# Daniel-Liu-c0deb0t/block-aligner

Hardware: AMD Instinct MI355X
Metric: GCUPS (DP cells/s) on 10 kbp DNA X-drop batch; bit-exact score+CIGAR vs AVX2 (higher is better)
Workload: dtype i16 (saturating lane scores) + i32 block offsets

## Files before the change

### block_aligner_amd/csrc/ba_driver.hpp

```cpp
#pragma once
#include "ba_device.hpp"

namespace ba {

#ifndef BA_BIG
#define BA_BIG 0
#endif
constexpr bool kBig = BA_BIG != 0;
__device__ __forceinline__ void lds_sync() {
    if (kBig) __builtin_amdgcn_fence(__ATOMIC_ACQ_REL, "workgroup");
    else __builtin_amdgcn_fence(__ATOMIC_ACQ_REL, "wavefront");
    __builtin_amdgcn_wave_barrier();
}
__device__ __forceinline__ void lds_fill0(short* a, uint32_t n) {
    for (uint32_t k = 2 * lane_id(); k < n; k += 128) *(int*)(a + k) = 0;
    lds_sync();
}
__device__ __forceinline__ void lds_copy(short* dst, const short* src, uint32_t n) {
    lds_sync();
    for (uint32_t k = 2 * lane_id(); k < n; k += 128) {
        const int v = *(const int*)(src + k);
        lds_sync();
        *(int*)(dst + k) = v;
    }
// ... 1692 lines not shown
                    pf_ok = false;
                    prev_dir = DIR_GROW;
                    block_size /= 2;
                    lds_copy(L.D_col, L.D_col + block_size, block_size); lds_copy(L.C_col, L.C_col + block_size, block_size);
                    lds_copy(L.D_row, L.D_row + block_size, block_size); lds_copy(L.R_row, L.R_row + block_size, block_size);
                    si += block_size; sj += block_size;
                    park<0>(parked, (int)si); park<1>(parked, (int)sj); park<2>(parked, off);
                    save_ckpt_borders(block_size);
                    right_max = lds_prefix_max8(L.D_col);
                    down_max = lds_prefix_max8(L.D_row);
                    if (TRACE) { park<3>(parked, (int)trace_top); park<4>(parked, (int)nblocks); }
                    y_drop_iter = 0;
                }
            }
            if (down_max > right_max) { si += STEP; dir = DIR_DOWN; }
            else { sj += STEP; dir = DIR_RIGHT; }
        }

        BA_TSTAMP(tr1);
        BA_TADD(prof, 15, tr0, tr1);
#ifdef BA_TIMING
        prof[16] += steps;
#endif
        if (TRACE && XDROP && chain && coldp()->prof) {
            uint32_t sc = 0;
            const uint32_t first = ub_nb < nblocks ? ub_nb : nblocks;
            for (uint32_t k = first + (uint32_t)lane_id(); k < nblocks; k += 64u) {
                const uint32_t* rp = (const uint32_t*)(blocks + k);
                const uint32_t hw = __hip_atomic_load(rp + 2, BA_RLX_AGENT), tb = __hip_atomic_load(rp + 3, BA_RLX_AGENT);
                if (tb & 0x40000000u) sc += (hw & 0xffffu) * (hw >> 16);
            }
#pragma unroll
            for (int d = 32; d >= 1; d >>= 1) sc += (uint32_t)__shfl_xor((int)sc, d, 64);
            if (is_lane(0) && sc) atomicAdd(coldp()->prof + 60, (unsigned long long)sc);
        }
        const uint32_t pair = (uint32_t)unpark<7>(parked), slot = (uint32_t)unpark<8>(parked);
        int score; uint32_t ri, rj;
        if (XDROP || FQE) { score = best_max; ri = (uint32_t)unpark<5>(parked); rj = (uint32_t)unpark<6>(parked); }
        else {
            lds_sync();
            if (dir == DIR_DOWN) score = off + uni((int)L.D_row[rlen - sj]) - ZERO;
            else score = off + uni((int)L.D_col[qlen - si]) - ZERO;
            ri = qlen; rj = rlen;
        }
        uint32_t ncig = 0;
        if (TRACE && batch_traceback) {
            if (is_lane(0)) {
                coldp()->score[pair] = score; coldp()->query_idx[pair] = ri; coldp()->reference_idx[pair] = rj;
                if (coldp()->cells) coldp()->cells[pair] = cells;
                if (coldp()->nblocks_out) coldp()->nblocks_out[pair] = nblocks;
                if (coldp()->trace_words_out) coldp()->trace_words_out[pair] = trace_top;
            }
            hand_off(slot, pair, ri, rj);
            return mout;
        }
        const bool walk_later = TRACE && coldp()->trace_off && qlen + rlen < coldp()->inline_len2 && !(MULTI && walk_now && !SPECIAL);
        if (TRACE && coldp()->cig_ops && !status && !walk_later) {
            __builtin_amdgcn_fence(__ATOMIC_SEQ_CST, "agent");
            if constexpr (SPECIAL) {
                if (is_lane(0)) {
                    uint32_t st = 0;
                    ncig = traceback(blocks, nblocks, trace, ri, rj, q, r, h_flags, coldp()->cig_ops, coldp()->cig_off[pair], coldp()->cig_off[pair + 1], &st);
                    status |= st;
                }
            } else {
                uint32_t st = 0;
                lds_sync();
// ... 245 lines not shown
```

### block_aligner_amd/csrc/ba_host.cpp

```cpp
#include <hip/hip_runtime.h>

#include <algorithm>
#include <functional>
#include <cmath>
#include <cstdarg>
#include <cstdio>
#include <cstdlib>
#include <cstring>
#include <map>
#include <memory>
#include <string>
#include <vector>
#include <atomic>
#include <chrono>
#include <thread>

#include "../../include/block_aligner_hip.h"
#include "aa_matrices.inc"
#include "ba_launch.h"

using ba::BatchParams;
using ba::BlockRec;

typedef const ba::KernelEntry* KernelTable[2][ba::N_KINDS][ba::N_CLASSES][ba::FAM_COUNT];
// ... 1707 lines not shown
    HIP_TRY(hipSetDevice(b->device));
    if (b->compacted && b->retried == 0) {
        const unsigned long long total = *(volatile unsigned long long*)b->h_total;
        if (total <= b->compact_used_cap) {
            if (total > capacity) return fail("cigar buffer too small: need %llu entries", total);
            if (b->compact_host) { if (runs != b->compact_host && total) memcpy(runs, b->compact_host, total * 4); }
            else if (total) HIP_TRY(hipMemcpy(runs, b->compact.p, total * 4, hipMemcpyDeviceToHost));
            return 0;
        }
    }
    std::vector<uint32_t> len(b->n);
    if (d2h(b->cig_len, len.data(), b->n)) return 1;
    std::vector<uint64_t> out_off(b->n);
    uint64_t total = 0;
    if (b->h_order.empty()) for (uint32_t p = 0; p < b->n; p++) { out_off[p] = total; total += len[p]; }
    else {
        std::vector<uint32_t> dev_of(b->n);
        for (uint32_t s = 0; s < b->n; s++) dev_of[b->h_order[s]] = s;
        for (uint32_t p = 0; p < b->n; p++) { out_off[dev_of[p]] = total; total += len[dev_of[p]]; }
    }
    if (total > capacity) return fail("cigar buffer too small: need %llu entries", (unsigned long long)total);
    if (total == 0) return 0;
    DevBuf d_off, d_out;
    if (d_off.alloc(b->n * 8) || d_out.alloc(total * 4)) return 1;
    HIP_TRY(hipMemcpy(d_off.p, out_off.data(), b->n * 8, hipMemcpyHostToDevice));
    HIP_TRY(ba_launch_compact_cigars(b->stream, b->cig_ops.as<uint32_t>(), b->cig_off.as<uint64_t>(), b->cig_len.as<uint32_t>(),
                                     d_off.as<uint64_t>(), d_out.as<uint32_t>(), b->n));
    HIP_TRY(hipStreamSynchronize(b->stream));
    HIP_TRY(hipMemcpy(runs, d_out.p, total * 4, hipMemcpyDeviceToHost));
    return 0;
}
#ifdef BA_DEV
int ba_dev_lane_scan(int form, const int16_t* x, uint32_t n_cells, int gap_extend, int16_t* out) {
    if (form < 0 || form > 4 || !x || !out) return fail("ba_dev_lane_scan: bad arguments");
    const uint32_t per_wave = form <= 1 ? 512u : (form == 2 ? 128u : (form == 3 ? 64u : 32u));
    if (n_cells == 0 || n_cells % per_wave) return fail("ba_dev_lane_scan: %u cells are not whole waves of %u", n_cells, per_wave);
    if (gap_extend > 0 || gap_extend < -128) return fail("ba_dev_lane_scan: gap_extend %d", gap_extend);
    DevBuf dx, dout;
    if (dx.alloc((size_t)n_cells * 2) || dout.alloc((size_t)n_cells * 2)) return 1;
    HIP_TRY(hipMemcpy(dx.p, x, (size_t)n_cells * 2, hipMemcpyHostToDevice));
    HIP_TRY(ba_launch_lane_kat(nullptr, form, dx.as<short>(), dout.as<short>(), gap_extend, n_cells / per_wave));
    HIP_TRY(hipDeviceSynchronize());
    HIP_TRY(hipMemcpy(out, dout.p, (size_t)n_cells * 2, hipMemcpyDeviceToHost));
    return 0;
}
int ba_dev_kernel_forms(int family, int kind, int pclass, int special) {
    const ba::KernelEntry* k = find_kernel(family, kind, pclass, special);
    return !k ? 0 : (k->fn[1][0][0] ? 2 : 1);
}
#endif
int ba_batch_prof(BaBatch* b, uint64_t out[128]) {
    if (!b) return fail("null batch");
    HIP_TRY(hipMemcpy(out, b->prof.p, 1024, hipMemcpyDeviceToHost));
    return 0;
}
int ba_batch_info(BaBatch* b, uint64_t out[4]) {
    if (!b) return fail("null batch");
    out[0] = (uint64_t)b->grid * b->wpw; out[1] = b->lds / b->wpw; out[2] = b->trace.bytes; out[3] = b->pool_bytes;
    return 0;
}
int ba_batch_spec_cells(BaBatch* b, uint64_t* cells) {
    if (!b || !cells) return fail("null argument");
    if (!b->ran) return fail("ba_batch_run has not been called");
    HIP_TRY(hipSetDevice(b->device));
    HIP_TRY(hipMemcpy(cells, (const char*)b->prof.p + 60 * 8, 8, hipMemcpyDeviceToHost));
    return 0;
}
int ba_batch_kernel(BaBatch* b) {
// ... 975 lines not shown
```

### block_aligner_amd/csrc/ba_kernels.hip

```cpp
#include "ba_driver.hpp"
#include "ba_launch.h"

#ifndef BA_KIND
#error "define BA_KIND"
#endif
#ifndef BA_PMAX
#error "define BA_PMAX"
#endif

#ifndef BA_SPECIAL
#define BA_SPECIAL 0
#endif

#if !BA_BIG && (BA_KIND != 3 || (!BA_SPECIAL && BA_PMAX <= 8))
#include "ba_multi.hpp"
#endif
#if !BA_BIG && BA_PMAX <= 8 && (BA_KIND != 3 || !BA_SPECIAL)
#include "ba_small.hpp"
#endif
#if !BA_BIG && BA_PMAX == 1 && !BA_SPECIAL
#include "ba_quad.hpp"
#endif

#define K_ALIGN(T, X) ba::k_align<BA_PMAX, BA_KIND, T, X, (BA_SPECIAL != 0)>
// ... 31 lines not shown
    BA_ENTRY(ba::FAM_SMALL, ba::WAVES_PER_WG, K_SMALL),
#endif
#if BA_SPECIAL && !BA_BIG && BA_KIND != 3
    BA_ENTRY_SPM(ba::FAM_MULTI, ba::WAVES_PER_WG, K_MULTI_S1, K_MULTI_S2),
#endif
#if BA_SPECIAL && !BA_BIG && BA_PMAX <= 8 && BA_KIND != 3
    BA_ENTRY_SPM(ba::FAM_SMALL, ba::WAVES_PER_WG, K_SMALL_S1, K_SMALL_S2),
#endif
#if BA_PMAX == 1 && !BA_SPECIAL && !BA_BIG
    {ba::FAM_QUAD, ba::WAVES_PER_WG, ba::lds_table_bytes_h(BA_KIND) + ba::WAVES_PER_WG * 4 * ba::QUAD_SLOT_BYTES, {BA_TX(K_QUAD), {}}},
#endif
};
[[maybe_unused]] static const int g_registered = ba::register_kernels(BA_KIND, BA_PMAX, BA_SPECIAL != 0, g_entries, (int)(sizeof g_entries / sizeof g_entries[0]));

#if BA_KIND == 0 && BA_PMAX == 1 && !BA_SPECIAL && !BA_BIG
__global__ void __launch_bounds__(64) k_traceback(const ba::BatchParams bp) {
    using namespace ba;
    __shared__ uint32_t words[4096];
    uint32_t st = 0, n = 0;
    if (bp.flags & (F_LOCAL | F_FQS)) {
        if (lane_id() == 0)
            n = traceback(bp.blocks + (uint64_t)bp.tb_slot * bp.blocks_stride, bp.tb_nblocks, bp.trace_arena + (uint64_t)bp.tb_slot * bp.trace_stride, bp.tb_i,
                          bp.tb_j, bp.pool + bp.q_off[0], bp.pool + bp.r_off[0], bp.flags, bp.cig_ops, bp.cig_off[0], bp.cig_off[1], &st);
    } else
        n = walk_wave<false>(bp.blocks + (uint64_t)bp.tb_slot * bp.blocks_stride, bp.tb_nblocks, bp.trace_arena + (uint64_t)bp.tb_slot * bp.trace_stride, bp.tb_i,
                             bp.tb_j, bp.pool + bp.q_off[0], bp.pool + bp.r_off[0], (bp.flags & F_CIGAR_EQ) != 0, bp.cig_ops, bp.cig_off[0], bp.cig_off[1], &st,
                             words, 4096u);
    if (lane_id() == 0) { bp.cig_len[0] = n; bp.status[0] = st; }
}

__global__ void __launch_bounds__(64) k_lane_kat(int form, const short* __restrict__ x, short* __restrict__ out, int gap_extend) {
    using namespace ba;
    const int lane = lane_id();
    if (form <= 1) {
        const short* xi = x + (size_t)blockIdx.x * 512 + lane * 8;
        int xr[4], r[4];
#pragma unroll
        for (int k = 0; k < 4; k++) xr[k] = pk((int)xi[2 * k], (int)xi[2 * k + 1]);
        const int ge2 = splat(gap_extend);
#pragma unroll
        for (int k = 0; k < 4; k++) r[k] = scan8_inreg(xr[k], ge2);
        int G[4], cs;
        if (form == 0) {
            const MultiConsts mc = make_multi_consts(lane & 15, gap_extend);
#pragma unroll
            for (int k = 0; k < 4; k++) G[k] = mc.G[k];
            scan8_chain(r, G[0]);
            cs = multi_carry(r[3], mc);
        } else {
            const SmallConsts mc = make_small_consts(lane & 3, gap_extend);
#pragma unroll
            for (int k = 0; k < 4; k++) G[k] = mc.G[k];
            scan8_chain(r, G[0]);
            cs = small_carry(r[3], mc, lane & 3);
        }
        short* oi = out + (size_t)blockIdx.x * 512 + lane * 8;
#pragma unroll
        for (int k = 0; k < 4; k++) { const int v = scan8_apply(r[k], cs, G[k], k == 3); oi[2 * k] = as_s(v).x; oi[2 * k + 1] = as_s(v).y; }
    } else {
        const int nl = form == 2 ? 64 : (form == 3 ? 32 : 16);
        const size_t base = (size_t)blockIdx.x * (size_t)(2 * nl);
        const int xv = lane < nl ? pk((int)x[base + 2 * lane], (int)x[base + 2 * lane + 1]) : 0;
        const FillConsts fc = make_fill_consts(lane, 0, gap_extend);
        const int v = form == 2 ? fast_scan<64>(xv, fc) : (form == 3 ? fast_scan<32>(xv, fc) : fast_scan<16>(xv, fc));
        if (lane < nl) { out[base + 2 * lane] = as_s(v).x; out[base + 2 * lane + 1] = as_s(v).y; }
    }
}
extern "C" hipError_t ba_launch_lane_kat(hipStream_t s, int form, const short* x, short* out, int gap_extend, unsigned waves) {
    k_lane_kat<<<dim3(waves), dim3(64), 0, s>>>(form, x, out, gap_extend);
    return hipGetLastError();
}

constexpr int WALK_WAVES = 4;
__global__ void __launch_bounds__(WALK_WAVES * 64) k_walk(const ba::BatchParams bp) {
    extern __shared__ __attribute__((aligned(16))) unsigned char walk_lds[];
    ba::traceback_all(bp, (uint32_t)ba::F_CIGAR_EQ, walk_lds + ((uint32_t)threadIdx.x >> 6) * ba::TB_LDS_BYTES);
}

__global__ void __launch_bounds__(WALK_WAVES * 64) k_walk_l2(const ba::BatchParams bp) {
// ... 134 lines not shown
```

### block_aligner_amd/csrc/ba_multi.hpp

```cpp
#pragma once
#include "ba_quad.hpp"

namespace ba {
#ifndef MQ_SOLO_PRIO
#define MQ_SOLO_PRIO 2
#endif

template <int N>
__device__ __forceinline__ int row_bcast(int v) { return __builtin_amdgcn_update_dpp(v, v, 0x150 + N, 0xf, 0xf, false); }
__device__ __forceinline__ int row_shl1_keep(int last, int src) { return __builtin_amdgcn_update_dpp(last, src, 0x101, 0xf, 0xf, false); }
__device__ __forceinline__ int splat_hi(int x) { const s16x2 t = as_s(x); return as_i(s16x2{t.y, t.y}); }
__device__ __forceinline__ int splat_lo(int x) { const s16x2 t = as_s(x); return as_i(s16x2{t.x, t.x}); }

__device__ __forceinline__ int sel_mask(unsigned long long m, int a, int b) {
    int r;
    asm("v_cndmask_b32_e64 %0, %1, %2, %3" : "=v"(r) : "v"(b), "v"(a), "s"(m));
    return r;
}

template <int SL> __device__ __forceinline__ int slot_first(int v) {
    if constexpr (SL == 16) return row_bcast<0>(v);
    else if constexpr (SL == 64) return __builtin_amdgcn_readfirstlane(v);
    else return __builtin_amdgcn_ds_bpermute((lane_id() & 32) << 2, v);
}
template <int SL> __device__ __forceinline__ int slot_last(int v) {
    if constexpr (SL == 16) return row_bcast<15>(v);
    else if constexpr (SL == 64) return __builtin_amdgcn_readlane(v, 63);
    else return __builtin_amdgcn_ds_bpermute(((lane_id() & 32) + 31) << 2, v);
}
template <int SL> __device__ __forceinline__ int slot_shr1_z(int v, int l) {
    if constexpr (SL == 16) return row_shr1_z(v);
    else if constexpr (SL == 64) return wave_shr1_z(v);
    else { const int t = wave_shr1_z(v); return l == 0 ? 0 : t; }
}
template <int SL> __device__ __forceinline__ int slot_shl1_keep(int last, int src, int l) {
    if constexpr (SL == 16) return row_shl1_keep(last, src);
    else { const int t = __builtin_amdgcn_update_dpp(last, src, 0x130, 0xf, 0xf, false); return l == SL - 1 ? last : t; }
}

struct MultiConsts {
    int G[4];
    int laneKG, lanem1KG;
    int w0;
};

__device__ __forceinline__ MultiConsts make_multi_consts(int l, int gx) {
    MultiConsts mc;
    mc.laneKG = l * 8 * gx; mc.lanem1KG = l ? (l - 1) * 8 * gx : -32768;
#pragma unroll
    for (int k = 0; k < 4; k++) mc.G[k] = pk(max(-32768, (2 * k + 1) * gx), max(-32768, (2 * k + 2) * gx));
    mc.w0 = pk(0, l == 0 ? 0 : ((l & 1) ? max(-32768, 8 * l * gx) : 4 * gx));
    return mc;
}
template <int SL = 16>
__device__ __forceinline__ int multi_carry(int r3, const MultiConsts& mc, int l = 0) {
    if constexpr (SL == 16) {
        const int pm = wave_prefix_max16((int)as_s(r3).y - mc.laneKG);
        return vmax(scan8_splat_lo(add_row_shr1(pm, mc.lanem1KG)), mc.w0);
    } else {
        const int pm = SL == 64 ? wave_prefix_max((int)as_s(r3).y - mc.laneKG) : wave_prefix_max32((int)as_s(r3).y - mc.laneKG);
        const int cin = add_shr1(pm, mc.lanem1KG);
        return vmax(scan8_splat_lo(l == 0 ? -32768 : cin), mc.w0);
    }
}

struct MultiOut { int mx, act_max8, pas_max8, corner_new; };

template <int KIND, bool TRACE, int SPM = 0, int SL = 16>
__device__ __forceinline__ void multi_rect(const char* table, const FillConsts& fc, const MultiConsts& mc, int l, int (&Ad)[4], int (&Ac)[4],
                                           int (&Pd)[4], int (&Pr)[4], uint2 vb, uint32_t cb_lo, uint32_t cb_hi, int corner, int off_add,
                                           uint32_t* __restrict__ tout, bool store, MultiOut& o, int rz2 = 0, bool fqs_row0 = false, int* zout = nullptr) {
    uint32_t zacc[2] = {0, 0};
    const int offa = splat(off_add);
    int d[4], c[4], pd[4], pr[4];
#pragma unroll
    for (int k = 0; k < 4; k++) {
        d[k] = adds(Ad[k], offa); c[k] = adds(Ac[k], offa); pd[k] = adds(Pd[k], offa); pr[k] = adds(Pr[k], offa);
    }
    o.corner_new = slot_first<SL>(pd[3]) >> 16;
    ScoreKey<KIND> key[4];
#pragma unroll
    for (int k = 0; k < 4; k++) {
        const uint32_t w = k < 2 ? vb.x : vb.y;
        key[k] = make_key<KIND>((int)((w >> (16 * (k & 1))) & 0xffu), (int)((w >> (16 * (k & 1) + 8)) & 0xffu));
    }
    uint32_t kb[4] = {0, 0, 0, 0}, cbs_lo = 0, cbs_hi = 0;
    if constexpr (KIND == KIND_NUC) {
        const uint32_t tb = (uint32_t)(uintptr_t)table, k01 = nuc_keys2(vb.x), k23 = nuc_keys2(vb.y);
        kb[0] = add_word(k01, tb, 0); kb[1] = add_word(k01, tb, 1); kb[2] = add_word(k23, tb, 0); kb[3] = add_word(k23, tb, 1);
        cbs_lo = nuc_col_offsets(cb_lo); cbs_hi = nuc_col_offsets(cb_hi);
    }
    int dmax[4] = {0, 0, 0, 0}, tacc[8] = {0, 0, 0, 0, 0, 0, 0, 0};
    int nvD[4] = {0, 0, 0, 0}, nvR[4] = {0, 0, 0, 0};
    int holdD = 0, holdR = 0;
#pragma unroll
    for (int j = 0; j < STEP; j++) {
        const int cb = (int)(((j < 4 ? cb_lo : cb_hi) >> (8 * (j & 3))) & 0xffu);
        int sc[4];
#pragma unroll
        for (int k = 0; k < 4; k++) {
            if constexpr (KIND == KIND_NUC) sc[k] = lds_read_i32(add_byte(j < 4 ? cbs_lo : cbs_hi, kb[k], j));
            else sc[k] = fetch_score<KIND>(table, key[k], cb);
        }
        int prev = slot_shr1_z<SL>(d[3], l);
        if (j == 0) prev = l == 0 ? (int)((uint32_t)corner << 16) : prev;
        int d00[4];
        d00[0] = __builtin_amdgcn_alignbit(d[0], prev, 16);
#pragma unroll
        for (int k = 1; k < 4; k++) d00[k] = __builtin_amdgcn_alignbit(d[k], d[k - 1], 16);
        int d11[4], copen[4], cn[4], x[4], r[4];
#pragma unroll
        for (int k = 0; k < 4; k++) {
            d11[k] = adds(d00[k], sc[k]);
            if (SPM == 2 && k == 0) d11[0] = fqs_row0 ? (int)(((uint32_t)d11[0] & 0xffff0000u) | ((uint32_t)rz2 & 0xffffu)) : d11[0];
            if (SPM == 1) d11[k] = vmax(d11[k], rz2);
            copen[k] = adds(d[k], fc.go2);
            cn[k] = vmax(adds(c[k], fc.ge2), copen[k]);
            d11[k] = vmax(d11[k], cn[k]);
            x[k] = adds(d11[k], fc.ome2);
            r[k] = scan8_inreg(x[k], fc.ge2);
        }
        scan8_chain(r, mc.G[0]);
        const int cs = multi_carry<SL>(r[3], mc, l);
        int dn[4];
        uint32_t sC[4], sR[4], sCo[4], sRo[4];
#pragma unroll
        for (int k = 0; k < 4; k++) {
            r[k] = scan8_apply(r[k], cs, mc.G[k], k == 3);
            dn[k] = vmax(d11[k], r[k]);
            if (TRACE) {
                sC[k] = (uint32_t)subs(cn[k], dn[k]); sR[k] = (uint32_t)subs(r[k], dn[k]); sCo[k] = (uint32_t)subs(copen[k], cn[k]); sRo[k] = (uint32_t)subs(x[k], r[k]);
            }
            dmax[k] = vmax(dmax[k], dn[k]);
            d[k] = dn[k]; c[k] = cn[k];
        }
        if (TRACE && SPM == 1) {
#pragma unroll
            for (int p2 = 0; p2 < 2; p2++) {
                const uint32_t pZ = (uint32_t)__builtin_amdgcn_perm(subs(rz2, dn[2 * p2 + 1]), subs(rz2, dn[2 * p2]), 0x0b0a0908);
                zacc[p2] |= pZ & (0x01010101u << j);
            }
        }
        if (TRACE) {
#pragma unroll
            for (int p2 = 0; p2 < 2; p2++) {
                const uint32_t pC = (uint32_t)__builtin_amdgcn_perm((int)sC[2 * p2 + 1], (int)sC[2 * p2], 0x0b0a0908), pR = (uint32_t)__builtin_amdgcn_perm((int)sR[2 * p2 + 1], (int)sR[2 * p2], 0x0b0a0908);
                const uint32_t pCo = (uint32_t)__builtin_amdgcn_perm((int)sCo[2 * p2 + 1], (int)sCo[2 * p2], 0x0b0a0908), pRo = (uint32_t)__builtin_amdgcn_perm((int)sRo[2 * p2 + 1], (int)sRo[2 * p2], 0x0b0a0908);
                const uint32_t lo2 = bfi(0x55555555u, pC, pR), hi2 = bfi(0x55555555u, pCo, pRo);
                const uint32_t nib = bfi(0x33333333u, lo2, hi2);
                if (j & 1) tacc[2 * (j >> 1) + p2] = (int)bfi(0xF0F0F0F0u, nib, (uint32_t)tacc[2 * (j >> 1) + p2]);
                else tacc[2 * (j >> 1) + p2] = (int)nib;
            }
        }
        if (j & 1) { nvD[j >> 1] = __builtin_amdgcn_perm(dn[3], holdD, 0x07060302); nvR[j >> 1] = __builtin_amdgcn_perm(r[3], holdR, 0x07060302); }
        else { holdD = dn[3]; holdR = r[3]; }
    }
    if (TRACE) {
#ifndef MQ_X_NOTRSTORE
        if (store) { *(int4*)tout = int4{tacc[0], tacc[1], tacc[2], tacc[3]}; *(int4*)(tout + 4) = int4{tacc[4], tacc[5], tacc[6], tacc[7]}; }
#else
        asm volatile("" :: "v"(tacc[0]), "v"(tacc[1]), "v"(tacc[2]), "v"(tacc[3]), "v"(tacc[4]), "v"(tacc[5]), "v"(tacc[6]), "v"(tacc[7]));
#endif
    }
#pragma unroll
    for (int k = 0; k < 4; k++) {
        Pd[k] = slot_shl1_keep<SL>(nvD[k], pd[k], l); Pr[k] = slot_shl1_keep<SL>(nvR[k], pr[k], l);
        Ad[k] = d[k]; Ac[k] = c[k];
    }
    {
        const int ma = vmax(vmax(d[0], d[1]), vmax(d[2], d[3])), mb = vmax(vmax(Pd[0], Pd[1]), vmax(Pd[2], Pd[3]));
        const s16x2 sa = as_s(ma), sb = as_s(mb);
        const int xa = vmax(ma, as_i(s16x2{sa.y, sa.x})), xb = vmax(mb, as_i(s16x2{sb.y, sb.x}));
        const s16x2 rr = as_s(slot_first<SL>(__builtin_amdgcn_perm(xb, xa, 0x05040100)));
        o.act_max8 = rr.x; o.pas_max8 = rr.y;
    }
    const int mm = vmax(vmax(dmax[0], dmax[1]), vmax(dmax[2], dmax[3]));
    const int m32 = max(mm & 0xffff, (int)((uint32_t)mm >> 16));
    o.mx = slot_last<SL>(SL == 16 ? wave_prefix_max16(m32) : (SL == 64 ? wave_prefix_max(m32) : wave_prefix_max32(m32)));
    if constexpr (TRACE && SPM == 1) { zout[0] = (int)~zacc[0]; zout[1] = (int)~zacc[1]; }
}

enum { MR_PAIR = 0, MR_BEST_I, MR_BEST_J, MR_CELLS_LO, MR_CELLS_HI, MR_BUDGET, MR_STATUS, MR_TSLOT, MR_SI, MR_SJ, MR_DIR, MR_PREV_DIR, MR_OFF, MR_OFF_MAX,
       MR_BEST_MAX, MR_Y_DROP, MR_X_ITER, MR_D_CORNER, MR_NSTEPS, MR_TRACE_TOP, MR_NBLOCKS, MR_SEL, MR_WORDS };
__device__ __forceinline__ int mq_load(const char* p) { return __hip_atomic_load((const int*)p, BA_RLX_AGENT); }

#ifndef MQ_PARTIAL_MB
#define MQ_PARTIAL_MB 256
#endif
#ifndef MQ_WAVES_EU
#define MQ_WAVES_EU 4
#endif
template <int PMAX, int KIND, bool TRACE, bool XDROP, int SPM = 0, int MBP = 128, int WPW = WAVES_PER_WG, int EU = MQ_WAVES_EU>
__global__ void __launch_bounds__(WPW * 64, (PMAX >= 16 ? 2 : EU)) k_multi(const BatchParams bp) {
    constexpr uint32_t MB = (uint32_t)MBP;
    constexpr int SL = MBP / 8, NSLOT = 64 / SL;
    constexpr uint32_t ALLM = (1u << NSLOT) - 1u;
    constexpr uint32_t ARR = 2u * MB, BUFL = 4u * ARR, BUFA = BUFL + 64u, SLOTA = 2u * BUFA + 128u;
    static_assert((MBP == 128 || MBP == 256 || MBP == 512) && NSLOT * SLOTA <= MQ_WAVE_BYTES && NSLOT * 2u * BUFL <= MQ_LDS_SCALARS && (MBP == 128 || SPM == 0), "k_multi slot geometry");
    static_assert(MBP != 128 || (BUFA == MQ_BUF_BYTES && SLOTA == MQ_SLOT_BYTES), "ba_params.h");
    constexpr uint32_t MQ_TW = (STEP * MB / 8) * (SPM == 1 ? 2u : 1u);
    constexpr int TB_LB = SPM ? (int)TB_LANE_BYTES_LOC : (int)TB_LANE_BYTES_L2;
    constexpr uint32_t TB_MASK = SPM ? ~0u : (uint32_t)F_CIGAR_EQ;
    extern __shared__ __attribute__((aligned(16))) char smem[];
    const int lane = lane_id(), l = lane & (SL - 1), g = lane / SL;
    const int wave = uni((int)threadIdx.x >> 6);
    {
        char* tab = smem;
        if (KIND == KIND_NUC) {
            nuc_table_fill(tab, bp.matrix, (int)threadIdx.x, WPW * 64);
        } else {
            const int nbytes = KIND == KIND_AA ? 27 * 32 : 2;
            for (int k = (int)threadIdx.x; k < nbytes; k += WPW * 64) tab[k] = (char)bp.matrix[k];
// ... 286 lines not shown
            } else live_m &= ~(1u << solo);
#ifdef BA_TIMING
            t_solo += __builtin_amdgcn_s_memtime() - ts_a; n_solo++;
#endif
        }
        if (!live_m) break;

        {
            BA_TSTAMP(tq_a);
            char* const slot_mem = wave_mem + (uint32_t)g * SLOTA;
            const int x_drop = bp.x_drop;
            FillConsts fq;
            fq.go2 = splat(bp.gap_open); fq.ge2 = splat(gx); fq.ome2 = splat(clamp16(bp.gap_open - gx));
            MultiConsts mc = make_multi_consts(l, gx);
            const uint64_t tcap64 = bp.trace_stride, bcap64 = bp.blocks_stride;
            const uint32_t tcap = (uint32_t)(tcap64 < 0x7fffffffull ? tcap64 : 0x7fffffffull), bcap = (uint32_t)(bcap64 < 0x7fffffffull ? bcap64 : 0x7fffffffull);
            const bool live = (live_m >> g) & 1u;
            const char* rec = slot_mem + 2 * BUFA;
#define BA_R(k) (live ? mq_load(rec + 4 * (k)) : 0)
            const uint32_t pair = (uint32_t)BA_R(MR_PAIR), tslot = (uint32_t)BA_R(MR_TSLOT);
            uint32_t si = (uint32_t)BA_R(MR_SI), sj = (uint32_t)BA_R(MR_SJ), y_drop = (uint32_t)BA_R(MR_Y_DROP);
            uint32_t trace_top = (uint32_t)BA_R(MR_TRACE_TOP), nblocks = (uint32_t)BA_R(MR_NBLOCKS), sel = (uint32_t)BA_R(MR_SEL);
            int dir = BA_R(MR_DIR), prev_dir = BA_R(MR_PREV_DIR), off = BA_R(MR_OFF), off_max = BA_R(MR_OFF_MAX), best_max = BA_R(MR_BEST_MAX);
            int x_iter = BA_R(MR_X_ITER), D_corner = BA_R(MR_D_CORNER);
#undef BA_R
            int A_d[4], A_c[4], P_d[4], P_r[4];
            {
                const char* b = slot_mem + (sel ^ 1u) * BUFA + l * 16;
#pragma unroll
                for (int k = 0; k < 4; k++) {
                    A_d[k] = live ? mq_load(b + 4 * k) : 0; A_c[k] = live ? mq_load(b + ARR + 4 * k) : 0;
                    P_d[k] = live ? mq_load(b + 2 * ARR + 4 * k) : 0; P_r[k] = live ? mq_load(b + 3 * ARR + 4 * k) : 0;
                }
            }
            char* const lbuf = base + (uint32_t)g * (2u * BUFL);
            int* const lsc = (int*)(base + MQ_LDS_SCALARS) + (uint32_t)g * MQ_LSC_INTS;
            lds_sync();
            const unsigned long long qa_r = TRACE ? 0ull : (unsigned long long)(bp.pool + (live ? bp.q_off[pair] : 0ull)), ra_r = TRACE ? 0ull : (unsigned long long)(bp.pool + (live ? bp.r_off[pair] : 0ull));
            const uint32_t qlen_r = (!TRACE && live) ? bp.q_len[pair] : 0u, rlen_r = (!TRACE && live) ? bp.r_len[pair] : 0u;
            if (TRACE && l == 0) {
                const unsigned long long qa = (unsigned long long)(bp.pool + (live ? bp.q_off[pair] : 0ull)), ra = (unsigned long long)(bp.pool + (live ? bp.r_off[pair] : 0ull));
                *(int4*)(lsc + 20) = int4{(int)(uint32_t)qa, (int)(uint32_t)(qa >> 32), (int)(uint32_t)ra, (int)(uint32_t)(ra >> 32)};
                *(int4*)(lsc + 24) = int4{live ? (int)bp.q_len[pair] : 0, live ? (int)bp.r_len[pair] : 0, (int)tslot, 0};
            }
            if (live) {
                const char* cb = slot_mem + sel * BUFA;
                char* d = lbuf + sel * BUFL + l * 16;
#pragma unroll
                for (int a = 0; a < 4; a++) {
                    const char* sp = cb + a * ARR + l * 16;
                    *(int4*)(d + a * ARR) = int4{mq_load(sp), mq_load(sp + 4), mq_load(sp + 8), mq_load(sp + 12)};
                }
                if (l < 9) lsc[sel * 9u + l] = mq_load(cb + BUFL + 4 * l);
            }
            lds_sync();
            uint2 pf_qv = {0, 0}, pf_rv = {0, 0}, pf_qc = {0, 0}, pf_rc = {0, 0}; bool pf_ok = false;
            bool leave = false;
            auto stage = [&](uint32_t which, uint32_t s_i, uint32_t s_j, int s_off, uint32_t s_tt, uint32_t s_nb, int s_dir, int s_offadd, int s_corner) {
                char* b = lbuf + which * BUFL + l * 16;
                *(int4*)(b) = int4{A_d[0], A_d[1], A_d[2], A_d[3]}; *(int4*)(b + ARR) = int4{A_c[0], A_c[1], A_c[2], A_c[3]};
                *(int4*)(b + 2 * ARR) = int4{P_d[0], P_d[1], P_d[2], P_d[3]}; *(int4*)(b + 3 * ARR) = int4{P_r[0], P_r[1], P_r[2], P_r[3]};
                if (l == 0) {
                    int* sc = lsc + which * 9u;
                    sc[0] = 1; sc[1] = (int)s_i; sc[2] = (int)s_j; sc[3] = s_off; sc[4] = (int)s_tt; sc[5] = (int)s_nb; sc[6] = s_dir; sc[7] = s_offadd; sc[8] = s_corner;
                }
            };
            do {
                const bool right = dir == DIR_RIGHT;
                int4 cA = {0, 0, 0, 0}, cB = {0, 0, 0, 0};
                if (TRACE) { cA = *(const int4*)(lsc + 20); cB = *(const int4*)(lsc + 24); }
                const uint8_t* const qp = TRACE ? (const uint8_t*)((unsigned long long)(uint32_t)cA.x | ((unsigned long long)(uint32_t)cA.y << 32)) : (const uint8_t*)qa_r;
                const uint8_t* const rp = TRACE ? (const uint8_t*)((unsigned long long)(uint32_t)cA.z | ((unsigned long long)(uint32_t)cA.w << 32)) : (const uint8_t*)ra_r;
                const uint32_t qlen = TRACE ? (uint32_t)cB.x : qlen_r, rlen = TRACE ? (uint32_t)cB.y : rlen_r;
                const uint32_t ri = right ? si : sj, rj = (right ? sj : si) + (MB - STEP);
                const uint32_t lenV = right ? qlen : rlen, lenC = right ? rlen : qlen;
                const bool q_out = si + MB > qlen, r_out = sj + MB > rlen;
                bool elig = XDROP || ri + MB <= lenV || rj + STEP <= lenC;
                if (TRACE) elig = elig && nblocks < bcap && trace_top + MQ_TW + 64 <= tcap;
                leave = live && !elig;
                const bool run = live && !leave;
                const int off_n = off_max;
                const int off_add = sat16(off - off_n);
                const int corner = (prev_dir != dir && prev_dir != DIR_GROW) ? sat16(D_corner + off_add) : 0;
#ifndef MQ_X_NOSTAGE
                if (live) stage(sel ^ 1u, si, sj, off_n, trace_top, nblocks, dir, off_add, corner);
#endif
                asm volatile("" : "+v"(mc.laneKG), "+v"(mc.lanem1KG), "+v"(mc.w0));
                uint32_t l8;
                asm volatile("v_mbcnt_lo_u32_b32 %0, -1, 0\n\tv_mbcnt_hi_u32_b32 %0, -1, %0" : "=v"(l8));
                l8 = (l8 & (uint32_t)(SL - 1)) * 8u;
                uint2 vb, cbv;
                {
                    const uint8_t* Vp = right ? qp : rp; const uint8_t* Cp = right ? rp : qp;
                    vb = right ? pf_qv : pf_rv; cbv = right ? pf_rc : pf_qc;
                    if (__any(run && !pf_ok)) {
                        if (run && !pf_ok) {
                            const uint32_t* vp = (const uint32_t*)(Vp + (ri + l8));
                            vb.x = vp[0]; vb.y = vp[1];
                            const uint32_t* cp = (const uint32_t*)(Cp + rj);
                            cbv.x = cp[0]; cbv.y = cp[1];
                        }
                    }
                    asm volatile("" : "+v"(vb.x), "+v"(vb.y));
                    if (run) {
                        const uint32_t* a = (const uint32_t*)(qp + (si + l8)); const uint32_t* b = (const uint32_t*)(rp + (sj + l8));
                        const uint32_t* cq = (const uint32_t*)(qp + si + MB); const uint32_t* cr = (const uint32_t*)(rp + sj + MB);
                        pf_qv.x = a[0]; pf_qv.y = a[1]; pf_rv.x = b[0]; pf_rv.y = b[1];
                        pf_qc.x = cq[0]; pf_qc.y = cq[1]; pf_rc.x = cr[0]; pf_rc.y = cr[1];
                        pf_ok = true;
                    }
                }
                uint32_t* tw = nullptr;
                if (TRACE) {
                    uint32_t ts = (uint32_t)cB.z; asm volatile("" : "+v"(ts));
                    tw = bp.trace_arena + (uint64_t)ts * bp.trace_stride + (trace_top + l8);
                    if (run && l == 0) {
                        BlockRec br;
                        br.i = (right ? ri : rj) | 0x80000000u;
                        br.j = right ? rj : ri; br.h = (uint16_t)(right ? MB : STEP); br.w = (uint16_t)(right ? STEP : MB);
                        br.trace_base = trace_top | (right ? 0x80000000u : 0u);
                        bp.blocks[(uint64_t)(uint32_t)cB.z * bp.blocks_stride + nblocks] = br;
                    }
                }
// ... 5 lines not shown

                const int right_max = right ? o.act_max8 : o.pas_max8, down_max = right ? o.pas_max8 : o.act_max8;
                const int new_off_max = off_n + o.mx - ZERO;
                const bool improve = new_off_max > best_max;
                const uint32_t new_y = improve ? 0u : y_drop + 1;
                bool stop = q_out && r_out;
                if (XDROP) stop = stop || (!improve && new_off_max < best_max - x_drop && x_iter >= 1);
                stop = stop || (!q_out && !r_out && 2 * MB <= max_size && new_y > MB / STEP - 1);
                const bool commit = run && !stop;
                leave = leave || (run && stop);
                {
                    const bool imp = commit && improve;
                    if (keep_pre) sel ^= imp ? 1u : 0u;
                    best_max = imp ? new_off_max : best_max;
                    off = commit ? off_n : off; off_max = commit ? new_off_max : off_max; y_drop = commit ? new_y : y_drop;
                    prev_dir = commit ? dir : prev_dir; D_corner = commit ? o.corner_new : D_corner;
                    if (TRACE) { trace_top += commit ? MQ_TW : 0u; nblocks += commit ? 1u : 0u; }
                    if (XDROP) x_iter = commit ? ((new_off_max < best_max - x_drop) ? x_iter + 1 : 0) : x_iter;
                    const bool go_down = r_out || (!q_out && down_max > right_max);
                    si += (commit && go_down) ? (uint32_t)STEP : 0u; sj += (commit && !go_down) ? (uint32_t)STEP : 0u;
                    const int ndir = go_down ? DIR_DOWN : DIR_RIGHT;
                    const unsigned long long swap_m = __ballot(ndir != dir);
#pragma unroll
                    for (int k = 0; k < 4; k++) {
                        const int td = A_d[k], tc = A_c[k];
                        A_d[k] = sel_mask(swap_m, P_d[k], td); A_c[k] = sel_mask(swap_m, P_r[k], tc); P_d[k] = sel_mask(swap_m, td, P_d[k]); P_r[k] = sel_mask(swap_m, tc, P_r[k]);
                    }
                    dir = commit ? ndir : dir;
                }
#ifdef BA_TIMING
                n_quad++;
#endif
            } while (!__any(leave));
            if (live && !leave) stage(sel ^ 1u, si, sj, 0, trace_top, nblocks, dir, 0, 0);
            lds_sync();
            if (live) {
#pragma unroll
                for (int w = 0; w < 2; w++) {
                    const char* sp = lbuf + w * BUFL + l * 16;
                    char* d = slot_mem + w * BUFA + l * 16;
#pragma unroll
                    for (int a = 0; a < 4; a++) *(int4*)(d + a * ARR) = *(const int4*)(sp + a * ARR);
                    if (l < 9) *(int*)(slot_mem + w * BUFA + BUFL + 4 * l) = lsc[w * 9 + l];
                }
            }
            lds_sync();
            if (live && l == 0) {
                int* rc = (int*)(slot_mem + 2 * BUFA);
                const uint32_t nsteps = (uint32_t)mq_load((const char*)(rc + MR_NSTEPS)) + ((si + sj) - (uint32_t)mq_load((const char*)(rc + MR_SI)) - (uint32_t)mq_load((const char*)(rc + MR_SJ))) / (uint32_t)STEP;
                rc[MR_SI] = (int)si; rc[MR_SJ] = (int)sj; rc[MR_DIR] = dir; rc[MR_PREV_DIR] = prev_dir; rc[MR_OFF] = off; rc[MR_OFF_MAX] = off_max; rc[MR_BEST_MAX] = best_max;
                rc[MR_Y_DROP] = (int)y_drop; rc[MR_X_ITER] = x_iter; rc[MR_D_CORNER] = D_corner; rc[MR_NSTEPS] = (int)nsteps; rc[MR_TRACE_TOP] = (int)trace_top;
                rc[MR_NBLOCKS] = (int)nblocks; rc[MR_SEL] = (int)sel;
            }
            const unsigned long long lm = __ballot(leave && l == 0);
            pend_m = 0;
#pragma unroll
            for (int sl_i = 0; sl_i < NSLOT; sl_i++) pend_m |= (uint32_t)((lm >> (sl_i * SL)) & 1ull) << sl_i;
#ifdef BA_TIMING
            t_quad += __builtin_amdgcn_s_memtime() - tq_a;
#endif
        }
    }
#ifdef BA_TIMING
    if (bp.prof && is_lane(0)) {
        atomicMax(bp.prof + 40, (unsigned long long)__builtin_amdgcn_s_memrealtime());
        atomicAdd(bp.prof + 50, t_solo); atomicAdd(bp.prof + 51, t_quad); atomicAdd(bp.prof + 52, t_wait); atomicAdd(bp.prof + 53, n_solo); atomicAdd(bp.prof + 54, n_quad); atomicAdd(bp.prof + 55, 1ull);
    }
#endif
#ifdef BA_ENDHIST
    if (bp.prof && is_lane(0)) {
        const unsigned long long t0 = __hip_atomic_load(bp.prof + 43, BA_RLX_AGENT), t = __builtin_amdgcn_s_memrealtime();
        const unsigned long long k = t0 && t > t0 ? (t - t0) / 400000ull : 0ull;
        atomicAdd(bp.prof + 64 + (k < 63ull ? k : 63ull), 1ull);
        atomicMax(bp.prof + 40, t);
    }
#endif
// ... 23 lines not shown
```

Measured before the change: 2267.

## Split lane cells into even/odd half-words and restructure multi-slot scan

Changes the in-register layout of each lane's eight i16 cells so each packed register holds two cells four apart (split/join at load/store boundaries). The prefix scan along the column becomes a cross-register chain with a short cross-half fix-up, replacing the per-register in-register scan plus chain and apply steps. This should cut ALU and permute work in the hot block step. The trace packing, the key extraction and the column-value extraction are re-permuted to match. It also rewrites LDS staging through explicit address-space-3 pointers and recomputes lane addresses inside the loop. Risks include layout mismatches that would break bit-exactness.

After: 2338, median of 6. +3.1%, better.

```diff
diff --git a/block_aligner_amd/csrc/ba_driver.hpp b/block_aligner_amd/csrc/ba_driver.hpp
--- a/block_aligner_amd/csrc/ba_driver.hpp
+++ b/block_aligner_amd/csrc/ba_driver.hpp
@@ -1748,7 +1748,7 @@
             }
 #pragma unroll
             for (int d = 32; d >= 1; d >>= 1) sc += (uint32_t)__shfl_xor((int)sc, d, 64);
-            if (is_lane(0) && sc) atomicAdd(coldp()->prof + 60, (unsigned long long)sc);
+            if (is_lane(0) && sc && !(status & ST_CLASS_OVERFLOW)) atomicAdd(coldp()->prof + 60, (unsigned long long)sc);
         }
         const uint32_t pair = (uint32_t)unpark<7>(parked), slot = (uint32_t)unpark<8>(parked);
         int score; uint32_t ri, rj;
diff --git a/block_aligner_amd/csrc/ba_host.cpp b/block_aligner_amd/csrc/ba_host.cpp
--- a/block_aligner_amd/csrc/ba_host.cpp
+++ b/block_aligner_amd/csrc/ba_host.cpp
@@ -1763,8 +1763,8 @@
 }
 #ifdef BA_DEV
 int ba_dev_lane_scan(int form, const int16_t* x, uint32_t n_cells, int gap_extend, int16_t* out) {
-    if (form < 0 || form > 4 || !x || !out) return fail("ba_dev_lane_scan: bad arguments");
-    const uint32_t per_wave = form <= 1 ? 512u : (form == 2 ? 128u : (form == 3 ? 64u : 32u));
+    if (form < 0 || form > 7 || !x || !out) return fail("ba_dev_lane_scan: bad arguments");
+    const uint32_t per_wave = (form <= 1 || form >= 5) ? 512u : (form == 2 ? 128u : (form == 3 ? 64u : 32u));
     if (n_cells == 0 || n_cells % per_wave) return fail("ba_dev_lane_scan: %u cells are not whole waves of %u", n_cells, per_wave);
     if (gap_extend > 0 || gap_extend < -128) return fail("ba_dev_lane_scan: gap_extend %d", gap_extend);
     DevBuf dx, dout;
diff --git a/block_aligner_amd/csrc/ba_kernels.hip b/block_aligner_amd/csrc/ba_kernels.hip
--- a/block_aligner_amd/csrc/ba_kernels.hip
+++ b/block_aligner_amd/csrc/ba_kernels.hip
@@ -87,6 +87,22 @@
 __global__ void __launch_bounds__(64) k_lane_kat(int form, const short* __restrict__ x, short* __restrict__ out, int gap_extend) {
     using namespace ba;
     const int lane = lane_id();
+    if (form >= 5) {
+        const short* xi = x + (size_t)blockIdx.x * 512 + lane * 8;
+        int r[4];
+#pragma unroll
+        for (int k = 0; k < 4; k++) r[k] = pk((int)xi[k], (int)xi[k + 4]);
+        const int ge2 = splat(gap_extend);
+        const int l = lane & (form == 5 ? 15 : (form == 6 ? 31 : 63));
+        const MultiConsts mc = make_multi_consts(l, gap_extend);
+        const int r3 = scan_halves(r, ge2, mc);
+        const int cs = form == 5 ? multi_carry<16>(r3, mc, l) : (form == 6 ? multi_carry<32>(r3, mc, l) : multi_carry<64>(r3, mc, l));
+        apply_halves(r, r3, cs, ge2, mc);
+        short* oi = out + (size_t)blockIdx.x * 512 + lane * 8;
+#pragma unroll
+        for (int k = 0; k < 4; k++) { oi[k] = as_s(r[k]).x; oi[k + 4] = as_s(r[k]).y; }
+        return;
+    }
     if (form <= 1) {
         const short* xi = x + (size_t)blockIdx.x * 512 + lane * 8;
         int xr[4], r[4];
@@ -99,7 +115,7 @@
         if (form == 0) {
             const MultiConsts mc = make_multi_consts(lane & 15, gap_extend);
 #pragma unroll
-            for (int k = 0; k < 4; k++) G[k] = mc.G[k];
+            for (int k = 0; k < 4; k++) G[k] = pk(max(-32768, (2 * k + 1) * gap_extend), max(-32768, (2 * k + 2) * gap_extend));
             scan8_chain(r, G[0]);
             cs = multi_carry(r[3], mc);
         } else {
diff --git a/block_aligner_amd/csrc/ba_multi.hpp b/block_aligner_amd/csrc/ba_multi.hpp
--- a/block_aligner_amd/csrc/ba_multi.hpp
+++ b/block_aligner_amd/csrc/ba_multi.hpp
@@ -38,8 +38,31 @@
     else { const int t = __builtin_amdgcn_update_dpp(last, src, 0x130, 0xf, 0xf, false); return l == SL - 1 ? last : t; }
 }
 
+__device__ __forceinline__ void cells_split(int (&v)[4]) {
+    const int a = v[0], b = v[1], c = v[2], d = v[3];
+    v[0] = __builtin_amdgcn_perm(c, a, 0x05040100); v[1] = __builtin_amdgcn_perm(c, a, 0x07060302);
+    v[2] = __builtin_amdgcn_perm(d, b, 0x05040100); v[3] = __builtin_amdgcn_perm(d, b, 0x07060302);
+}
+__device__ __forceinline__ void cells_join(int (&v)[4]) {
+    const int a = v[0], b = v[1], c = v[2], d = v[3];
+    v[0] = __builtin_amdgcn_perm(b, a, 0x05040100); v[1] = __builtin_amdgcn_perm(d, c, 0x05040100);
+    v[2] = __builtin_amdgcn_perm(b, a, 0x07060302); v[3] = __builtin_amdgcn_perm(d, c, 0x07060302);
+}
+__device__ __forceinline__ int4 cells_split(int4 q) { int v[4] = {q.x, q.y, q.z, q.w}; cells_split(v); return int4{v[0], v[1], v[2], v[3]}; }
+__device__ __forceinline__ int4 cells_join(int4 q) { int v[4] = {q.x, q.y, q.z, q.w}; cells_join(v); return int4{v[0], v[1], v[2], v[3]}; }
+__device__ __forceinline__ int adds_lo(int a, int k) {
+    int t;
+    asm("v_pk_add_i16 %0, %1, %2 op_sel_hi:[0,1] clamp" : "=v"(t) : "v"(a), "s"(k));
+    return t;
+}
+__device__ __forceinline__ int max_hi_lo(int a, int b) {
+    asm("v_max_i16_sdwa %0, %0, %1 dst_sel:WORD_1 dst_unused:UNUSED_PRESERVE src0_sel:WORD_1 src1_sel:WORD_0" : "+v"(a) : "v"(b));
+    return a;
+}
+
 struct MultiConsts {
-    int G[4];
+    int g2, g3;
+    int K4, G48;
     int laneKG, lanem1KG;
     int w0;
 };
@@ -47,8 +70,8 @@
 __device__ __forceinline__ MultiConsts make_multi_consts(int l, int gx) {
     MultiConsts mc;
     mc.laneKG = l * 8 * gx; mc.lanem1KG = l ? (l - 1) * 8 * gx : -32768;
-#pragma unroll
-    for (int k = 0; k < 4; k++) mc.G[k] = pk(max(-32768, (2 * k + 1) * gx), max(-32768, (2 * k + 2) * gx));
+    mc.g2 = splat(max(-32768, 2 * gx)); mc.g3 = splat(max(-32768, 3 * gx));
+    mc.K4 = pk(0, max(-32768, 4 * gx)); mc.G48 = pk(max(-32768, 4 * gx), max(-32768, 8 * gx));
     mc.w0 = pk(0, l == 0 ? 0 : ((l & 1) ? max(-32768, 8 * l * gx) : 4 * gx));
     return mc;
 }
@@ -64,6 +87,18 @@
     }
 }
 
+__device__ __forceinline__ int scan_halves(int (&r)[4], int ge2, const MultiConsts& mc) {
+#pragma unroll
+    for (int k = 1; k < 4; k++) r[k] = vmax(r[k], adds(r[k - 1], ge2));
+    return vmax(r[3], adds_lo(r[3], mc.K4));
+}
+__device__ __forceinline__ void apply_halves(int (&r)[4], int r3, int cs, int ge2, const MultiConsts& mc) {
+    const int t = max_hi_lo(adds_lo(cs, mc.K4), r[3]);
+    r[0] = vmax(r[0], adds(t, ge2)); r[1] = vmax(r[1], adds(t, mc.g2)); r[2] = vmax(r[2], adds(t, mc.g3));
+    r[3] = vmax(r3, adds(cs, mc.G48));
+}
+
+typedef int lds_v4i __attribute__((ext_vector_type(4)));
 struct MultiOut { int mx, act_max8, pas_max8, corner_new; };
 
 template <int KIND, bool TRACE, int SPM = 0, int SL = 16>
@@ -80,19 +115,17 @@
     o.corner_new = slot_first<SL>(pd[3]) >> 16;
     ScoreKey<KIND> key[4];
 #pragma unroll
-    for (int k = 0; k < 4; k++) {
-        const uint32_t w = k < 2 ? vb.x : vb.y;
-        key[k] = make_key<KIND>((int)((w >> (16 * (k & 1))) & 0xffu), (int)((w >> (16 * (k & 1) + 8)) & 0xffu));
-    }
+    for (int k = 0; k < 4; k++) key[k] = make_key<KIND>((int)((vb.x >> (8 * k)) & 0xffu), (int)((vb.y >> (8 * k)) & 0xffu));
     uint32_t kb[4] = {0, 0, 0, 0}, cbs_lo = 0, cbs_hi = 0;
     if constexpr (KIND == KIND_NUC) {
-        const uint32_t tb = (uint32_t)(uintptr_t)table, k01 = nuc_keys2(vb.x), k23 = nuc_keys2(vb.y);
+        const uint32_t tb = (uint32_t)(uintptr_t)table;
+        const uint32_t k01 = nuc_keys2((uint32_t)__builtin_amdgcn_perm((int)vb.y, (int)vb.x, 0x05010400)), k23 = nuc_keys2((uint32_t)__builtin_amdgcn_perm((int)vb.y, (int)vb.x, 0x07030602));
         kb[0] = add_word(k01, tb, 0); kb[1] = add_word(k01, tb, 1); kb[2] = add_word(k23, tb, 0); kb[3] = add_word(k23, tb, 1);
         cbs_lo = nuc_col_offsets(cb_lo); cbs_hi = nuc_col_offsets(cb_hi);
     }
     int dmax[4] = {0, 0, 0, 0}, tacc[8] = {0, 0, 0, 0, 0, 0, 0, 0};
     int nvD[4] = {0, 0, 0, 0}, nvR[4] = {0, 0, 0, 0};
-    int holdD = 0, holdR = 0;
+    int holdD[4] = {0, 0, 0, 0}, holdR[4] = {0, 0, 0, 0};
 #pragma unroll
     for (int j = 0; j < STEP; j++) {
         const int cb = (int)(((j < 4 ? cb_lo : cb_hi) >> (8 * (j & 3))) & 0xffu);
@@ -105,9 +138,9 @@
         int prev = slot_shr1_z<SL>(d[3], l);
         if (j == 0) prev = l == 0 ? (int)((uint32_t)corner << 16) : prev;
         int d00[4];
-        d00[0] = __builtin_amdgcn_alignbit(d[0], prev, 16);
-#pragma unroll
-        for (int k = 1; k < 4; k++) d00[k] = __builtin_amdgcn_alignbit(d[k], d[k - 1], 16);
+        d00[0] = __builtin_amdgcn_alignbit(d[3], prev, 16);
+#pragma unroll
+        for (int k = 1; k < 4; k++) d00[k] = d[k - 1];
         int d11[4], copen[4], cn[4], x[4], r[4];
 #pragma unroll
         for (int k = 0; k < 4; k++) {
@@ -118,15 +151,15 @@
             cn[k] = vmax(adds(c[k], fc.ge2), copen[k]);
             d11[k] = vmax(d11[k], cn[k]);
             x[k] = adds(d11[k], fc.ome2);
-            r[k] = scan8_inreg(x[k], fc.ge2);
-        }
-        scan8_chain(r, mc.G[0]);
-        const int cs = multi_carry<SL>(r[3], mc, l);
+            r[k] = x[k];
+        }
+        const int r3 = scan_halves(r, fc.ge2, mc);
+        const int cs = multi_carry<SL>(r3, mc, l);
+        apply_halves(r, r3, cs, fc.ge2, mc);
         int dn[4];
         uint32_t sC[4], sR[4], sCo[4], sRo[4];
 #pragma unroll
         for (int k = 0; k < 4; k++) {
-            r[k] = scan8_apply(r[k], cs, mc.G[k], k == 3);
             dn[k] = vmax(d11[k], r[k]);
             if (TRACE) {
                 sC[k] = (uint32_t)subs(cn[k], dn[k]); sR[k] = (uint32_t)subs(r[k], dn[k]); sCo[k] = (uint32_t)subs(copen[k], cn[k]); sRo[k] = (uint32_t)subs(x[k], r[k]);
@@ -137,23 +170,27 @@
         if (TRACE && SPM == 1) {
 #pragma unroll
             for (int p2 = 0; p2 < 2; p2++) {
-                const uint32_t pZ = (uint32_t)__builtin_amdgcn_perm(subs(rz2, dn[2 * p2 + 1]), subs(rz2, dn[2 * p2]), 0x0b0a0908);
+                const uint32_t pZ = (uint32_t)__builtin_amdgcn_perm(subs(rz2, dn[2 * p2 + 1]), subs(rz2, dn[2 * p2]), 0x0b090a08);
                 zacc[p2] |= pZ & (0x01010101u << j);
             }
         }
         if (TRACE) {
 #pragma unroll
             for (int p2 = 0; p2 < 2; p2++) {
-                const uint32_t pC = (uint32_t)__builtin_amdgcn_perm((int)sC[2 * p2 + 1], (int)sC[2 * p2], 0x0b0a0908), pR = (uint32_t)__builtin_amdgcn_perm((int)sR[2 * p2 + 1], (int)sR[2 * p2], 0x0b0a0908);
-                const uint32_t pCo = (uint32_t)__builtin_amdgcn_perm((int)sCo[2 * p2 + 1], (int)sCo[2 * p2], 0x0b0a0908), pRo = (uint32_t)__builtin_amdgcn_perm((int)sRo[2 * p2 + 1], (int)sRo[2 * p2], 0x0b0a0908);
+                const uint32_t pC = (uint32_t)__builtin_amdgcn_perm((int)sC[2 * p2 + 1], (int)sC[2 * p2], 0x0b090a08), pR = (uint32_t)__builtin_amdgcn_perm((int)sR[2 * p2 + 1], (int)sR[2 * p2], 0x0b090a08);
+                const uint32_t pCo = (uint32_t)__builtin_amdgcn_perm((int)sCo[2 * p2 + 1], (int)sCo[2 * p2], 0x0b090a08), pRo = (uint32_t)__builtin_amdgcn_perm((int)sRo[2 * p2 + 1], (int)sRo[2 * p2], 0x0b090a08);
                 const uint32_t lo2 = bfi(0x55555555u, pC, pR), hi2 = bfi(0x55555555u, pCo, pRo);
                 const uint32_t nib = bfi(0x33333333u, lo2, hi2);
                 if (j & 1) tacc[2 * (j >> 1) + p2] = (int)bfi(0xF0F0F0F0u, nib, (uint32_t)tacc[2 * (j >> 1) + p2]);
                 else tacc[2 * (j >> 1) + p2] = (int)nib;
             }
-        }
-        if (j & 1) { nvD[j >> 1] = __builtin_amdgcn_perm(dn[3], holdD, 0x07060302); nvR[j >> 1] = __builtin_amdgcn_perm(r[3], holdR, 0x07060302); }
-        else { holdD = dn[3]; holdR = r[3]; }
+            if (j & 1) {
+                const int wa = tacc[j - 1], wb = tacc[j];
+                tacc[j - 1] = __builtin_amdgcn_perm(wb, wa, 0x05040100); tacc[j] = __builtin_amdgcn_perm(wb, wa, 0x07060302);
+            }
+        }
+        if (j >= 4) { nvD[j - 4] = __builtin_amdgcn_perm(dn[3], holdD[j - 4], 0x07060302); nvR[j - 4] = __builtin_amdgcn_perm(r[3], holdR[j - 4], 0x07060302); }
+        else { holdD[j] = dn[3]; holdR[j] = r[3]; }
     }
     if (TRACE) {
 #ifndef MQ_X_NOTRSTORE
@@ -177,7 +214,7 @@
     const int mm = vmax(vmax(dmax[0], dmax[1]), vmax(dmax[2], dmax[3]));
     const int m32 = max(mm & 0xffff, (int)((uint32_t)mm >> 16));
     o.mx = slot_last<SL>(SL == 16 ? wave_prefix_max16(m32) : (SL == 64 ? wave_prefix_max(m32) : wave_prefix_max32(m32)));
-    if constexpr (TRACE && SPM == 1) { zout[0] = (int)~zacc[0]; zout[1] = (int)~zacc[1]; }
+    if constexpr (TRACE && SPM == 1) { zout[0] = ~__builtin_amdgcn_perm((int)zacc[1], (int)zacc[0], 0x05040100); zout[1] = ~__builtin_amdgcn_perm((int)zacc[1], (int)zacc[0], 0x07060302); }
 }
 
 enum { MR_PAIR = 0, MR_BEST_I, MR_BEST_J, MR_CELLS_LO, MR_CELLS_HI, MR_BUDGET, MR_STATUS, MR_TSLOT, MR_SI, MR_SJ, MR_DIR, MR_PREV_DIR, MR_OFF, MR_OFF_MAX,
@@ -530,16 +567,19 @@
                     A_d[k] = live ? mq_load(b + 4 * k) : 0; A_c[k] = live ? mq_load(b + ARR + 4 * k) : 0;
                     P_d[k] = live ? mq_load(b + 2 * ARR + 4 * k) : 0; P_r[k] = live ? mq_load(b + 3 * ARR + 4 * k) : 0;
                 }
+                cells_split(A_d); cells_split(A_c); cells_split(P_d); cells_split(P_r);
             }
             char* const lbuf = base + (uint32_t)g * (2u * BUFL);
+            constexpr uint32_t MQ_LSC_STATE = 9u, MQ_LSC_PAIR = 20u;
+            static_assert(2u * MQ_LSC_STATE <= MQ_LSC_PAIR && MQ_LSC_PAIR + 8u <= MQ_LSC_INTS && (4u * MQ_LSC_PAIR) % 16u == 0 && (4u * MQ_LSC_INTS) % 16u == 0, "a slot's scalars in LDS");
             int* const lsc = (int*)(base + MQ_LDS_SCALARS) + (uint32_t)g * MQ_LSC_INTS;
             lds_sync();
             const unsigned long long qa_r = TRACE ? 0ull : (unsigned long long)(bp.pool + (live ? bp.q_off[pair] : 0ull)), ra_r = TRACE ? 0ull : (unsigned long long)(bp.pool + (live ? bp.r_off[pair] : 0ull));
             const uint32_t qlen_r = (!TRACE && live) ? bp.q_len[pair] : 0u, rlen_r = (!TRACE && live) ? bp.r_len[pair] : 0u;
             if (TRACE && l == 0) {
                 const unsigned long long qa = (unsigned long long)(bp.pool + (live ? bp.q_off[pair] : 0ull)), ra = (unsigned long long)(bp.pool + (live ? bp.r_off[pair] : 0ull));
-                *(int4*)(lsc + 20) = int4{(int)(uint32_t)qa, (int)(uint32_t)(qa >> 32), (int)(uint32_t)ra, (int)(uint32_t)(ra >> 32)};
-                *(int4*)(lsc + 24) = int4{live ? (int)bp.q_len[pair] : 0, live ? (int)bp.r_len[pair] : 0, (int)tslot, 0};
+                *(int4*)(lsc + MQ_LSC_PAIR) = int4{(int)(uint32_t)qa, (int)(uint32_t)(qa >> 32), (int)(uint32_t)ra, (int)(uint32_t)(ra >> 32)};
+                *(int4*)(lsc + MQ_LSC_PAIR + 4) = int4{live ? (int)bp.q_len[pair] : 0, live ? (int)bp.r_len[pair] : 0, (int)tslot, 0};
             }
             if (live) {
                 const char* cb = slot_mem + sel * BUFA;
@@ -547,26 +587,38 @@
 #pragma unroll
                 for (int a = 0; a < 4; a++) {
                     const char* sp = cb + a * ARR + l * 16;
-                    *(int4*)(d + a * ARR) = int4{mq_load(sp), mq_load(sp + 4), mq_load(sp + 8), mq_load(sp + 12)};
-                }
-                if (l < 9) lsc[sel * 9u + l] = mq_load(cb + BUFL + 4 * l);
+                    *(int4*)(d + a * ARR) = cells_split(int4{mq_load(sp), mq_load(sp + 4), mq_load(sp + 8), mq_load(sp + 12)});
+                }
+                if ((uint32_t)l < MQ_LSC_STATE) lsc[sel * MQ_LSC_STATE + l] = mq_load(cb + BUFL + 4 * l);
             }
             lds_sync();
             uint2 pf_qv = {0, 0}, pf_rv = {0, 0}, pf_qc = {0, 0}, pf_rc = {0, 0}; bool pf_ok = false;
             bool leave = false;
-            auto stage = [&](uint32_t which, uint32_t s_i, uint32_t s_j, int s_off, uint32_t s_tt, uint32_t s_nb, int s_dir, int s_offadd, int s_corner) {
-                char* b = lbuf + which * BUFL + l * 16;
-                *(int4*)(b) = int4{A_d[0], A_d[1], A_d[2], A_d[3]}; *(int4*)(b + ARR) = int4{A_c[0], A_c[1], A_c[2], A_c[3]};
-                *(int4*)(b + 2 * ARR) = int4{P_d[0], P_d[1], P_d[2], P_d[3]}; *(int4*)(b + 3 * ARR) = int4{P_r[0], P_r[1], P_r[2], P_r[3]};
+            auto stage = [&](uint32_t lb, uint32_t ls, uint32_t which, uint32_t s_i, uint32_t s_j, int s_off, uint32_t s_tt, uint32_t s_nb, int s_dir, int s_offadd, int s_corner) {
+                typedef __attribute__((address_space(3))) lds_v4i* lds_int4_ptr;
+                typedef __attribute__((address_space(3))) int* lds_int_ptr;
+                const lds_int4_ptr b = (lds_int4_ptr)(uintptr_t)(lb + which * BUFL);
+                b[0] = lds_v4i{A_d[0], A_d[1], A_d[2], A_d[3]}; b[ARR / 16] = lds_v4i{A_c[0], A_c[1], A_c[2], A_c[3]};
+                b[2 * ARR / 16] = lds_v4i{P_d[0], P_d[1], P_d[2], P_d[3]}; b[3 * ARR / 16] = lds_v4i{P_r[0], P_r[1], P_r[2], P_r[3]};
                 if (l == 0) {
-                    int* sc = lsc + which * 9u;
+                    const lds_int_ptr sc = (lds_int_ptr)(uintptr_t)ls + which * MQ_LSC_STATE;
                     sc[0] = 1; sc[1] = (int)s_i; sc[2] = (int)s_j; sc[3] = s_off; sc[4] = (int)s_tt; sc[5] = (int)s_nb; sc[6] = s_dir; sc[7] = s_offadd; sc[8] = s_corner;
                 }
             };
+            const uint32_t base32 = (uint32_t)(uintptr_t)base;
             do {
                 const bool right = dir == DIR_RIGHT;
+                uint32_t lid;
+                asm volatile("v_mbcnt_lo_u32_b32 %0, -1, 0\n\tv_mbcnt_hi_u32_b32 %0, -1, %0" : "=v"(lid));
+                const uint32_t l8 = (lid & (uint32_t)(SL - 1)) * 8u;
+                const uint32_t lbuf_s = base32 + (lid / (uint32_t)SL) * (2u * BUFL) + 2u * l8;
+                const uint32_t lsc_s = base32 + (uint32_t)MQ_LDS_SCALARS + (lid / (uint32_t)SL) * (4u * (uint32_t)MQ_LSC_INTS);
                 int4 cA = {0, 0, 0, 0}, cB = {0, 0, 0, 0};
-                if (TRACE) { cA = *(const int4*)(lsc + 20); cB = *(const int4*)(lsc + 24); }
+                if (TRACE) {
+                    typedef const __attribute__((address_space(3))) lds_v4i* lds_cint4_ptr;
+                    const lds_v4i a4 = *(lds_cint4_ptr)(uintptr_t)(lsc_s + 4u * MQ_LSC_PAIR), b4 = *(lds_cint4_ptr)(uintptr_t)(lsc_s + 4u * (MQ_LSC_PAIR + 4u));
+                    cA = int4{a4.x, a4.y, a4.z, a4.w}; cB = int4{b4.x, b4.y, b4.z, b4.w};
+                }
                 const uint8_t* const qp = TRACE ? (const uint8_t*)((unsigned long long)(uint32_t)cA.x | ((unsigned long long)(uint32_t)cA.y << 32)) : (const uint8_t*)qa_r;
                 const uint8_t* const rp = TRACE ? (const uint8_t*)((unsigned long long)(uint32_t)cA.z | ((unsigned long long)(uint32_t)cA.w << 32)) : (const uint8_t*)ra_r;
                 const uint32_t qlen = TRACE ? (uint32_t)cB.x : qlen_r, rlen = TRACE ? (uint32_t)cB.y : rlen_r;
@@ -581,12 +633,9 @@
                 const int off_add = sat16(off - off_n);
                 const int corner = (prev_dir != dir && prev_dir != DIR_GROW) ? sat16(D_corner + off_add) : 0;
 #ifndef MQ_X_NOSTAGE
-                if (live) stage(sel ^ 1u, si, sj, off_n, trace_top, nblocks, dir, off_add, corner);
+                if (live) stage(lbuf_s, lsc_s, sel ^ 1u, si, sj, off_n, trace_top, nblocks, dir, off_add, corner);
 #endif
                 asm volatile("" : "+v"(mc.laneKG), "+v"(mc.lanem1KG), "+v"(mc.w0));
-                uint32_t l8;
-                asm volatile("v_mbcnt_lo_u32_b32 %0, -1, 0\n\tv_mbcnt_hi_u32_b32 %0, -1, %0" : "=v"(l8));
-                l8 = (l8 & (uint32_t)(SL - 1)) * 8u;
                 uint2 vb, cbv;
                 {
                     const uint8_t* Vp = right ? qp : rp; const uint8_t* Cp = right ? rp : qp;
@@ -658,7 +707,7 @@
                 n_quad++;
 #endif
             } while (!__any(leave));
-            if (live && !leave) stage(sel ^ 1u, si, sj, 0, trace_top, nblocks, dir, 0, 0);
+            if (live && !leave) stage((uint32_t)(uintptr_t)(lbuf + l * 16), (uint32_t)(uintptr_t)lsc, sel ^ 1u, si, sj, 0, trace_top, nblocks, dir, 0, 0);
             lds_sync();
             if (live) {
 #pragma unroll
@@ -666,8 +715,8 @@
                     const char* sp = lbuf + w * BUFL + l * 16;
                     char* d = slot_mem + w * BUFA + l * 16;
 #pragma unroll
-                    for (int a = 0; a < 4; a++) *(int4*)(d + a * ARR) = *(const int4*)(sp + a * ARR);
-                    if (l < 9) *(int*)(slot_mem + w * BUFA + BUFL + 4 * l) = lsc[w * 9 + l];
+                    for (int a = 0; a < 4; a++) *(int4*)(d + a * ARR) = cells_join(*(const int4*)(sp + a * ARR));
+                    if ((uint32_t)l < MQ_LSC_STATE) *(int*)(slot_mem + w * BUFA + BUFL + 4 * l) = lsc[w * MQ_LSC_STATE + l];
                 }
             }
             lds_sync();
```
